# ml4ai/iqlpref

Measured on AMD Instinct MI355X. Metric: iql_grad_steps_per_sec, higher is better.
Workload: dtype bf16; 1 GPU; IQL antmaze-medium-diverse-v2 shapes (S=29 A=8 H=256), 1M-transition device replay, batch 256, one seed per GPU; batch=256, buffer_rows=1000000, graph_unroll=0, graph_launches_per_block=0, eager_steps_per_block=1390

## Files before the change

iqlpref_amd/csrc/api.hip:

```cpp
#include <hip/hip_runtime.h>

#include <algorithm>
#include <cmath>
#include <cstdarg>
#include <cstdio>
#include <cstdlib>
#include <cstring>
#include <new>
#include <vector>

#include "../../include/iqlhip.h"
#include "common.h"
#include "iql_deep.h"
#include "iql_step.h"
#include "step_math.h"

namespace iqlhip {
struct DeepTrainer;
bool deep_shape_ok(const iqlhip_trainer_config &, int n_hidden, const char **why);
hipError_t deep_create(DeepTrainer **, const iqlhip_trainer_config &, int n_hidden, const iqlhip_arenas &,
                       const int64_t *offsets);
void deep_destroy(DeepTrainer *);
hipError_t deep_sync_weights(DeepTrainer *, hipStream_t);
const DeepDesc &deep_desc(const DeepTrainer *);
// ... 726 lines not shown
    TrainNet &N = D.net[n];
    N.in_dim = indim[n], N.k1pad = k1pad[n], N.out_dim = outdim[n], N.out_pad = outpad[n];
    N.has_target = n < E;
    for (int k = 0; k < 3; ++k) {
      N.off_w[k] = L.off[n * 6 + 2 * k];
      N.off_b[k] = L.off[n * 6 + 2 * k + 1];
      N.toff_w[k] = N.has_target ? N.off_w[k] : -1;
      N.toff_b[k] = N.has_target ? N.off_b[k] : -1;
    }
    N.wc[0] = carve<char>(p, (size_t)H * k1pad[n] * es);
    N.wc[1] = carve<char>(p, (size_t)H * H * es);
    N.wc[2] = carve<char>(p, (size_t)outpad[n] * H * es);
    if (N.has_target) {
      N.tc[0] = carve<char>(p, (size_t)H * k1pad[n] * es);
      N.tc[1] = carve<char>(p, (size_t)H * H * es);
      N.tc[2] = carve<char>(p, (size_t)outpad[n] * H * es);
    }
    N.w2ct = carve<char>(p, (size_t)H * H * es);
    N.w3t = carve<char>(p, (size_t)H * outpad[n] * es);
  }
  D.xT = carve<char>(p, (size_t)2 * D.xrows * D.BP * es);
  D.rd = carve<float>(p, (size_t)B * 2);
  D.actf = carve<float>(p, (size_t)B * A);
  D.hT = carve<char>(p, (size_t)NT * 2 * H * D.BP * es);
  D.dz1T = carve<char>(p, (size_t)NT * H * D.BP * es);
  D.dz2T = carve<char>(p, (size_t)NT * H * D.BP * es);
  D.dz3T = carve<char>(p, (size_t)NT * D.opmax * D.BP * es);
  D.outs = carve<float>(p, (size_t)layer2_parts(H) * B * D.OUTW);
  D.lossp = carve<float>(p, (size_t)NT * (B / 16));
  D.lsp = carve<float>(p, (size_t)(B / 16) * A);
  D.ls_snap = carve<float>(p, (size_t)A);
  t->batch_rows = carve<float>(p, (size_t)B * stride);
  D.stage_rows = carve<float>(p, (size_t)B * stride);
  D.stage_stride = stride;
  D.next_off = iqlhip_replay_next_offset(S, A);
  D.prefetch = !getenv("IQLHIP_NO_PREFETCH") ? 1 : 0;
  t->own_dargs = t->dargs = carve<DevArgs>(p, 1);
  t->own_dctr = t->dctr = carve<DevCtr>(p, 1);
  t->own_ddesc = t->ddesc = carve<TrainerDesc>(p, 1);
  t->own_ditems = t->ditems = carve<UpdItem>(p, n_slots);

  for (int n_ = 0; n_ < NT; ++n_)
  for (auto &it : t->net_items[n_]) {
    const TrainNet &N = D.net[it.net];
    const int L = it.layer;
    it.Odim = (L == 2) ? N.out_dim : H;
    it.Idim = (L == 0) ? N.in_dim : H;
    it.Opad = (L == 2) ? N.out_pad : H;
    it.Kw = (L == 0) ? N.k1pad : H;
    it.has_target = N.has_target;
    it.group = it.net == D.net_v ? 1 : (it.net == D.net_a ? 2 : 0);
    it.off_w = N.off_w[L], it.off_b = N.off_b[L], it.toff_w = N.toff_w[L], it.toff_b = N.toff_b[L];

    it.wc = N.wc[L], it.tc = N.has_target ? N.tc[L] : nullptr, it.w2ct = (L == 1) ? N.w2ct : nullptr;
    it.w3t = (L == 2) ? N.w3t : nullptr;
    const size_t plane = (size_t)H * D.BP * es;
    it.Xsrc = (L == 0) ? D.xT : reinterpret_cast<char *>(D.hT) + (size_t)(it.net * 2 + (L - 1)) * plane;
    it.Zsrc = (L == 0)   ? reinterpret_cast<char *>(D.dz1T) + (size_t)it.net * plane
              : (L == 1) ? reinterpret_cast<char *>(D.dz2T) + (size_t)it.net * plane
                         : reinterpret_cast<char *>(D.dz3T) + (size_t)it.net * D.opmax * D.BP * es;
  }
  std::vector<UpdItem> items;
  {
    std::vector<UpdItem> per_xcd[8];
    deal_items(t, 0, 1, per_xcd);
    items = flatten_table(per_xcd, 0, nullptr, (size_t)(B + 15) / 16);
  }
  if (items.size() != n_slots || hipMemcpy(t->ditems, items.data(), items.size() * sizeof(UpdItem), hipMemcpyHostToDevice) !=
      hipSuccess) {
    (void)hipFree(t->ws);
    delete t;
    return fail(IQLHIP_ERR_HIP, "hipMemcpy of the work items failed");
  }

  auto mk = [&](int f, int net, bool target, int in_off, int out_col, int slot) {
    FwdNet &F = D.fwd[f];
    const TrainNet &N = D.net[net];
    F.w1c = target ? N.tc[0] : N.wc[0];
    F.w2c = target ? N.tc[1] : N.wc[1];
    F.w3c = target ? N.tc[2] : N.wc[2];
    const float *base = target ? ar->target : ar->params;
    F.b1 = base + N.off_b[0], F.b2 = base + N.off_b[1], F.b3 = base + N.off_b[2];
    F.in_off = in_off, F.in_dim = N.in_dim, F.k1pad = N.k1pad;
    F.out_dim = N.out_dim, F.out_pad = N.out_pad, F.out_col = out_col;
    F.train_slot = slot;
    F.tanh_out = net == D.net_a;
    F.dropout = (net == D.net_a) && D.has_dropout;
    F.stage = f == 0;
  };
  for (int e = 0; e < E; ++e) mk(e, e, false, 0, e, e);
  mk(E, D.net_v, false, 0, D.out_v, D.net_v);
  mk(E + 1, D.net_a, false, 0, D.out_mean, D.net_a);
  for (int e = 0; e < E; ++e) mk(E + 2 + e, e, true, 0, D.out_qt + e, -1);
  mk(2 * E + 2, D.net_v, false, D.next_off, D.out_nv, -1);

  if (hipMemcpy(t->ddesc, &t->D, sizeof(TrainerDesc), hipMemcpyHostToDevice) != hipSuccess) {
    (void)hipFree(t->ws);
    delete t;
    return fail(IQLHIP_ERR_HIP, "hipMemcpy of the descriptor failed");
  }
  *out = t;
  return 0;
}

extern "C" int iqlhip_trainer_destroy(iqlhip_trainer *t) {
  if (!t) return 0;
  if (t->group) return fail(IQLHIP_ERR_INVALID, "trainer is a member of a group: destroy the group first");
  t->queue.destroy();
// ... 943 lines not shown
```

iqlpref_amd/csrc/iql_step.h:

```cpp
#pragma once
#include <stdint.h>

namespace iqlhip {

constexpr int MAX_CRITICS = 8;
constexpr int MAX_TRAIN = MAX_CRITICS + 2;
constexpr int MAX_FWD = 2 * MAX_CRITICS + 3;

struct FwdNet {
  const void *w1c, *w2c, *w3c;
  const float *b1, *b2, *b3;
  int32_t in_off;
  int32_t in_dim, k1pad;
  int32_t out_dim, out_pad;
  int32_t out_col;
  int32_t train_slot;
  int32_t tanh_out;
  int32_t dropout;
  int32_t stage;
};

struct TrainNet {
  int64_t off_w[3], off_b[3];
  int64_t toff_w[3], toff_b[3];
// ... 27 lines not shown
  float *actf;
  void *hT;
  void *dz1T;
  void *dz2T;
  void *dz3T;
  float *outs;
  float *lossp;
  float *lsp;
  float *ls_snap;
  float *params, *exp_avg, *exp_avg_sq, *target, *grads;
  int64_t off_log_std;
  unsigned long long *dbg;
  double beta1, beta2, eps;
  int64_t t_max;
  FwdNet fwd[MAX_FWD];
  TrainNet net[MAX_TRAIN];
};

struct DevArgs {
  const float *rows;
  int64_t n_rows;
  int32_t row_stride;
  int32_t idx_mode;
  const int64_t *idx;
  const uint8_t *drop_keep;
  float *losses_out;
  int64_t base_step;
  double lr_q, lr_v, lr_a_base;
  int64_t n_steps;
  uint64_t generation;
  const int32_t *n_valid;
};

struct AdamCoef {
  float one_m_b1, b2, one_m_b2, neg_step[3], bc2_sqrt, eps;
  float inv_bc2_sqrt, pad_;
};

struct DevCtr {
  int64_t ctr[2];
  int64_t coef_step;
  AdamCoef coef;
  float last_losses[4];
  double loss_sum[4];
};

struct UpdItem {
  int32_t net, layer;
  int32_t o0, i0;
  int32_t Odim, Idim;
  int32_t Opad, Kw;
  int32_t has_target, group;
  int64_t off_w, off_b, toff_w, toff_b;
  void *wc, *tc, *w2ct;
  void *w3t;
  const void *Xsrc, *Zsrc;
};

}
```

iqlpref_amd/csrc/iql_step.hip:

```cpp
#include "common.h"
#include "iql_step.h"
#include "step_math.h"

namespace iqlhip {

constexpr int SLAB = 16;

#ifdef IQL_STAMPS
#define STAMP(kern, slot)                                                                   \
  do {                                                                                      \
    if (D.dbg && threadIdx.x == 0 && blockIdx.x < 512) {                                                      \
      unsigned long long *d_ = D.dbg + (((size_t)(kern) * 512 + blockIdx.x) * 8 + (slot)) * 2; \
      d_[0] = wall_clock64();                                                               \
      d_[1] = clock64();                                                                    \
    }                                                                                       \
  } while (0)
#else
#define STAMP(kern, slot) \
  do {                    \
  } while (0)
#endif

template <class T>
__device__ __forceinline__ void pin_s(T v) {
// ... 274 lines not shown
          }
        }
      }
    }
  }
  STAMP(0, 5);
}

template <bool BF16>
__device__ __forceinline__ void stage_rows16(const TrainerDesc &D, const DevArgs &A, int64_t step, int row0,
                                             int row_step, int tid) {
  using P = Prec<BF16>;
  using T = typename P::T;
  const int rr = tid >> 4, l16 = tid & 15;
  const int B = D.B, nq = D.stage_stride >> 2, S = D.S, SA = D.S + D.A, nkb = D.BP / P::KM;
  T *const xT = reinterpret_cast<T *>(D.xT) + (size_t)(step & 1) * D.xrows * D.BP;
  for (int row = row0 + rr; row < B; row += row_step) {
    int64_t ix;
    if (A.idx_mode == 1)
      ix = ldg(A.idx + (size_t)(step - A.base_step) * B + row);
    else if (A.idx_mode == 2)
      ix = row;
    else
      ix = philox_index(D.seed, (uint64_t)step, (uint32_t)row, (uint64_t)A.n_rows);
    ix = ix < 0 ? 0 : (ix >= A.n_rows ? A.n_rows - 1 : ix);
    const float *src = A.rows + (size_t)ix * A.row_stride;
    float *dst = D.stage_rows + (size_t)row * D.stage_stride;
    for (int c = l16; c < nq; c += 16) {
      const float4 v4 = __builtin_bit_cast(float4, ldg16(src + 4 * c));
      stg16(dst + 4 * c, v4);
      const float v[4] = {v4.x, v4.y, v4.z, v4.w};
#pragma unroll
      for (int e = 0; e < 4; ++e) {
        const int col = 4 * c + e;
        if (col < SA) stg(xT + fidx<P>(col, row, nkb), P::from_f32(v[e]));
        if (col >= S && col < SA) stg(D.actf + (size_t)row * D.A + (col - S), v[e]);
        if (col >= SA && col < SA + 2) stg(D.rd + (size_t)row * 2 + (col - SA), v[e]);
      }
    }
  }
}

template <bool BF16>
__global__ __launch_bounds__(256) void k_stage(const TrainerDesc *__restrict__ Dp,
                                               const DevArgs *__restrict__ Ap,
                                               const DevCtr *__restrict__ Cp) {
  Dp += blockIdx.y, Ap += blockIdx.y, Cp += blockIdx.y;
  stage_rows16<BF16>(*Dp, *Ap, Cp->ctr[0], blockIdx.x * 16, gridDim.x * 16, threadIdx.x);
}

__device__ __forceinline__ void write_adam_coef(const TrainerDesc &D, const DevArgs &A, int64_t t1,
                                                AdamCoef *out);

template <bool BF16, int H>
struct FCfg {
  using P = Prec<BF16>;
  static constexpr int TPW = H / 64;
  static constexpr int SPL = TPW >= 4 ? 4 : TPW;
  static constexpr int HQ = H / SPL;
  static constexpr int NK2 = H / P::KM;
  static constexpr int NK3 = HQ / P::KM;
  static constexpr int NK1 = BF16 ? 4 : 8;
  static constexpr int HP = H + P::EPV;
  static constexpr int HQP = HQ + P::EPV;
  static_assert(HQ == 64, "one 16-column tile per wave and part");
};

template <bool BF16, int H, int MT, int PW>
__global__ __launch_bounds__(256, 3) void k_forward(const TrainerDesc *__restrict__ Dp,
                                                 const DevArgs *__restrict__ Ap,
                                                 const DevCtr *__restrict__ Cp, const int nsl_,
                                                 const int nfwd_) {
  using C = FCfg<BF16, H>;
  using P = Prec<BF16>;
  using T = typename P::T;
  constexpr int ROWS = 16 * MT, TPW = C::TPW, SPL = C::SPL, HP = C::HP, HQP = C::HQP;
  constexpr int NPG = SPL / PW;
  static_assert(SPL % PW == 0 && PW <= 2, "parts per work-group: 1 or 2, dividing the parts");
  Dp += blockIdx.y, Ap += blockIdx.y, Cp += blockIdx.y;
  const TrainerDesc &D = *Dp;
  const int idx_ = blockIdx.x >> 3;
  const int per_job = nsl_ * NPG;
  const int fnet = (idx_ / per_job) * 8 + (blockIdx.x & 7);
  const int rest = idx_ % per_job;
  const int slab = rest / NPG;
  const int part0 = __builtin_amdgcn_readfirstlane((rest % NPG) * PW);
  if (fnet > nfwd_) return;
  if (fnet == nfwd_) {
    if (rest == 0 && threadIdx.x == 0) {
      STAMP(0, 0);
      write_adam_coef(D, *Ap, Cp->ctr[0] + 1, const_cast<AdamCoef *>(&Cp->coef));
      const_cast<DevCtr *>(Cp)->coef_step = Cp->ctr[0] + 1;
      STAMP(0, 5);
    }
    if (rest == 0 && !D.deterministic && (int)threadIdx.x < D.A)
      stg(D.ls_snap + threadIdx.x, ldg(D.params + D.off_log_std + threadIdx.x));
    return;
  }
  const FwdNet N = D.fwd[fnet];
  const int B = D.B, BP = D.BP, OUTW = D.OUTW, k1max = D.k1max;
  const float *const stage = D.stage_rows;
  const unsigned sstride = (unsigned)D.stage_stride;
  float *const g_outs = D.outs;
  void *const g_hT = D.hT;
  const int64_t step = Cp->ctr[0];
  extern __shared__ __attribute__((aligned(16))) char smem[];
  const int tid = threadIdx.x, lane = tid & 63;
  const int wave = __builtin_amdgcn_readfirstlane(tid >> 6);
  const int r = lane & 15, q = lane >> 4;
  const int K1P = k1max + P::EPV;
  T *xs = reinterpret_cast<T *>(smem);
  T *h1 = xs + ROWS * K1P;
  T *h2 = h1 + ROWS * HP;
  STAMP(0, 0);

  const int rr = tid >> 4, l16 = tid & 15;
  const int lim4 = round_up(N.in_dim, 4) - 4;
  float4 xq[MT][2];
#pragma unroll
  for (int m = 0; m < MT; ++m) {
    const int row_ = slab * ROWS + 16 * m + rr;
    const unsigned row = (unsigned)(row_ < B ? row_ : B - 1);
    const float *src = stage + N.in_off;
#pragma unroll
    for (int j = 0; j < 2; ++j) {
      const int c = 4 * l16 + 64 * j;
      xq[m][j] = __builtin_bit_cast(float4, ldg16(src + (row * sstride + (unsigned)(c < lim4 ? c : lim4))));
    }
  }
  const int nk1 = N.k1pad / P::KM;
  const int nt3 = N.out_pad / 16;
  const int tile2 = part0 * 4 + wave;
  float bias1[TPW], bias3[2];
  {
    const float *b1w = N.b1 + 16 * (wave * TPW);
#pragma unroll
    for (int jj = 0; jj < TPW; ++jj) bias1[jj] = ldg(b1w + 16 * jj + r);
  }
  float bias2[PW];
#pragma unroll
  for (int j = 0; j < PW; ++j) bias2[j] = ldg(N.b2 + 16 * (tile2 + 4 * j) + r);
#pragma unroll
  for (int jt = 0; jt < 2; ++jt)
    bias3[jt] = ldg(N.b3 + (16 * jt + r < N.out_dim ? 16 * jt + r : N.out_dim - 1));
  uint4 w1[C::NK1][TPW], w2[PW][C::NK2], w3[PW][C::NK3][2];
  auto load_w2 = [&]() {
#pragma unroll
    for (int j = 0; j < PW; ++j) {
      const T *W2w = reinterpret_cast<const T *>(N.w2c) + (size_t)(tile2 + 4 * j) * C::NK2 * 64 * P::EPV;
#pragma unroll
      for (int ks = 0; ks < C::NK2; ++ks) w2[j][ks] = ldg16(W2w + ks * 64 * P::EPV + lane * P::EPV);
    }
  };
  auto load_w3 = [&]() {
#pragma unroll
    for (int j = 0; j < PW; ++j) {
      const T *W3w = reinterpret_cast<const T *>(N.w3c) + (size_t)((part0 + j) * C::NK3) * 64 * P::EPV;
#pragma unroll
      for (int ks = 0; ks < C::NK3; ++ks)
// ... 188 lines not shown

  for (int pr = wave; pr < MT * PW; pr += 4) {
    const int m = pr % MT, j = pr / MT;
    const T *h2j = h2 + j * ROWS * HQP;
    f32x4 acc3[2] = {f32x4{0.f, 0.f, 0.f, 0.f}, f32x4{0.f, 0.f, 0.f, 0.f}};
#pragma unroll
    for (int ks = 0; ks < C::NK3; ++ks) {
      const uint4 a = *reinterpret_cast<const uint4 *>(h2j + (16 * m + r) * HQP + ks * P::KM + P::EPV * q);
#pragma unroll
      for (int jt = 0; jt < 2; ++jt) {
        if (jt < nt3) {
          if constexpr (PW == 1) {
            P::mma(a, w3[0][ks][jt], acc3[jt]);
          } else {
            if (j == 0) P::mma(a, w3[0][ks][jt], acc3[jt]);
            else P::mma(a, w3[PW - 1][ks][jt], acc3[jt]);
          }
        }
      }
    }
    float *outp = g_outs + (size_t)(part0 + j) * B * OUTW;
    const int row0 = slab * ROWS + 16 * m + 4 * q;
#pragma unroll
    for (int jt = 0; jt < 2; ++jt) {
      const int col = 16 * jt + r;
      if (jt < nt3 && col < N.out_dim && row0 < B) {
        const float bias = part0 + j == 0 ? P::round(bias3[jt]) : 0.f;
        outs_store4<false>(outp, (size_t)(N.out_col + col) * B + row0,
                           make_float4(acc3[jt][0] + bias, acc3[jt][1] + bias, acc3[jt][2] + bias, acc3[jt][3] + bias));
      }
    }
  }
  STAMP(0, 5);
}

template <int H, bool DROP>
__global__ __launch_bounds__(512, 1) void k_forward_tp(const TrainerDesc *__restrict__ Dp,
                                                        const DevArgs *__restrict__ Ap,
                                                        const DevCtr *__restrict__ Cp, const int nsl_,
                                                        const int nfwd_) {
  using C = FCfg<true, H>;
  using P = Prec<true>;
  using T = typename P::T;
  constexpr int ROWS = 64, MT = ROWS / 16, NW = 8;
  constexpr int TPW = H / (16 * NW);
  constexpr int SPL = C::SPL, HP = C::HP, NK2 = C::NK2, NK3 = C::NK3;
  static_assert(H == 256 && TPW == 2 && SPL == 4, "k_forward_tp is built for H = 256");
  Dp += blockIdx.y, Ap += blockIdx.y, Cp += blockIdx.y;
  const TrainerDesc &D = *Dp;
  const int idx_ = blockIdx.x >> 3;
  const int fnet = (idx_ / nsl_) * 8 + (blockIdx.x & 7);
  const int slab = idx_ % nsl_;
  if (fnet > nfwd_) return;
  if (fnet == nfwd_) {
    if (slab == 0 && threadIdx.x == 0) {
      STAMP(0, 0);
      write_adam_coef(D, *Ap, Cp->ctr[0] + 1, const_cast<AdamCoef *>(&Cp->coef));
      const_cast<DevCtr *>(Cp)->coef_step = Cp->ctr[0] + 1;
      STAMP(0, 5);
    }
    if (slab == 0 && !D.deterministic && (int)threadIdx.x < D.A)
      stg(D.ls_snap + threadIdx.x, ldg(D.params + D.off_log_std + threadIdx.x));
    return;
  }
  const FwdNet N = D.fwd[fnet];
  const int B = D.B, BP = D.BP, OUTW = D.OUTW, k1max = D.k1max;
  const float *const stage = D.stage_rows;
  const unsigned sstride = (unsigned)D.stage_stride;
  float *const g_outs = D.outs;
  void *const g_hT = D.hT;
  const int64_t step = Cp->ctr[0];
  extern __shared__ __attribute__((aligned(16))) char smem[];
  const int tid = threadIdx.x, lane = tid & 63;
  const int wave = __builtin_amdgcn_readfirstlane(tid >> 6);
  const int r = lane & 15, q = lane >> 4;
  const int K1P = k1max + P::EPV;
  T *xs = reinterpret_cast<T *>(smem);
  T *h1 = xs + ROWS * K1P;
  T *h2 = h1 + ROWS * HP;
  STAMP(0, 0);

  const int rr = tid >> 3, l8 = tid & 7;
  const int lim4 = round_up(N.in_dim, 4) - 4;
  float4 xq[4];
  {
    const int row_ = slab * ROWS + rr;
    const unsigned row = (unsigned)(row_ < B ? row_ : B - 1);
    const float *src = stage + N.in_off;
#pragma unroll
    for (int j = 0; j < 4; ++j) {
      const int c = 4 * l8 + 32 * j;
      xq[j] = __builtin_bit_cast(float4, ldg16(src + (row * sstride + (unsigned)(c < lim4 ? c : lim4))));
    }
  }
  const int nk1 = N.k1pad / P::KM;
  const int nt3 = N.out_pad / 16;
  const int tile0 = wave * TPW;
  const int part = tile0 / 4;
  float bias1[TPW], bias2[TPW], bias3[2];
#pragma unroll
  for (int jj = 0; jj < TPW; ++jj) {
    bias1[jj] = ldg(N.b1 + 16 * (tile0 + jj) + r);
    bias2[jj] = ldg(N.b2 + 16 * (tile0 + jj) + r);
  }
#pragma unroll
  for (int jt = 0; jt < 2; ++jt)
    bias3[jt] = ldg(N.b3 + (16 * jt + r < N.out_dim ? 16 * jt + r : N.out_dim - 1));
  uint4 w1[C::NK1][TPW], w2[TPW][NK2], w3[NK3][2];
  {
    const T *W1w = reinterpret_cast<const T *>(N.w1c) + (size_t)tile0 * nk1 * 64 * P::EPV;
#pragma unroll
    for (int ks = 0; ks < C::NK1; ++ks) {
      if (ks < nk1) {
#pragma unroll
        for (int jj = 0; jj < TPW; ++jj)
          w1[ks][jj] = ldg16(W1w + (size_t)(jj * nk1 + ks) * 64 * P::EPV + lane * P::EPV);
      }
    }
  }
  auto load_w23 = [&]() {
#pragma unroll
    for (int jj = 0; jj < TPW; ++jj) {
      const T *W2w = reinterpret_cast<const T *>(N.w2c) + (size_t)(tile0 + jj) * NK2 * 64 * P::EPV;
#pragma unroll
      for (int ks = 0; ks < NK2; ++ks) w2[jj][ks] = ldg16(W2w + ks * 64 * P::EPV + lane * P::EPV);
// ... 850 lines not shown
      for (int s = 0; s < nslab; ++s) g += sred[nl + s * D.A + tid];
      const int64_t o = D.off_log_std + tid;
      const float lsc = fminf(fmaxf(ls, -20.f), 2.f);
      g = g * expf(lsc) * ((ls >= -20.f && ls <= 2.f) ? 1.f : 0.f);
      float p = ls;
      adam_apply<BF16>(p, pm, pv, g, coef, coef.neg_step[2]);
      stg(D.params + o, p), stg(D.exp_avg + o, pm), stg(D.exp_avg_sq + o, pv);
      if (D.grads) stg(D.grads + o, g);
    }
    if (tid >= 64 && tid < 64 + nt) {
      const int n = tid - 64;
      float s = 0.f;
      for (int k = 0; k < nslab; ++k) s += sred[n * nslab + k];
      int nv = B;
      if constexpr (!BF16) nv = VALID_ROWS(A.n_valid, A, t1 - 1, B);
      sred[nl + na + n] = s / (float)nv;
    }
    __syncthreads();
    if (tid == 64) {
      const float vl = sred[nl + na + D.net_v];
      float ql = 0.f;
      for (int e = 0; e < D.E; ++e) ql += sred[nl + na + e];
      ql = ql / (float)D.E;
      const float al = sred[nl + na + D.net_a];
      Cp->last_losses[0] = vl, Cp->last_losses[1] = ql, Cp->last_losses[2] = al;
      Cp->loss_sum[0] += vl, Cp->loss_sum[1] += ql, Cp->loss_sum[2] += al;
      if (A.losses_out) {
        float *lo = A.losses_out + (size_t)(t1 - 1 - A.base_step) * 3;
        stg(lo, vl), stg(lo + 1, ql), stg(lo + 2, al);
      }
      Cp->ctr[0] = t1;
    }
    STAMP(2, 4);
    return;
  }

  if (it.net < 0) {
    if (D.prefetch && (A.idx_mode == 0 || (A.idx_mode == 1 && t1 - A.base_step < A.n_steps)))
      stage_rows16<BF16>(D, A, t1, it.o0 * (UT / 16), it.i0 * (UT / 16), tid);
    return;
  }
  const int L = it.layer;
  const int Odim = it.Odim, Idim = it.Idim, Kw = it.Kw, Opad = it.Opad;
  const int Ipad = round_up(Idim, 16);
  const int o0 = it.o0, i0 = it.i0;
  const float neg_step =
      it.group == 0 ? coef.neg_step[0] : (it.group == 1 ? coef.neg_step[1] : coef.neg_step[2]);
  const bool has_target = it.has_target != 0;
  const int nk = BP / P::KM;
  const int kh = (BF16 && nk >= 16) ? (nk / (2 * UKC)) * UKC : nk;
  const bool ksplit = kh < nk;
  pin_s(D.tau), pin_s(D.one_m_tau), pin_s(D.polyak_convex);
  pin_s(it.off_w), pin_s(it.toff_w), pin_s(it.off_b), pin_s(it.toff_b), pin_s(it.wc), pin_s(it.tc);
  pin_s(it.w2ct), pin_s(it.Xsrc), pin_s(it.Zsrc), pin_s(Kw), pin_s(neg_step);
  pin_s(coef.one_m_b1), pin_s(coef.b2), pin_s(coef.one_m_b2), pin_s(coef.bc2_sqrt), pin_s(coef.eps);
  pin_s(coef.inv_bc2_sqrt);

  if (L == 0) {
    const int TLD = Ipad + 4;
    const int64_t fbase = it.off_w + (int64_t)o0 * Idim, tbase = it.toff_w + (int64_t)o0 * Idim;
    constexpr int UNE = LAT ? (USR * UMAXI + UT - 1) / UT : 1;
    constexpr int UN4 = LAT ? 1 : (USR * UMAXI / 4 + UT - 1) / UT;
    const int n_el = USR * Idim, n4 = n_el >> 2;
    float pf[UNE], mf[UNE], vf[UNE], tf[UNE];
    float4 pf4[UN4], mf4[UN4], vf4[UN4], tf4[UN4];
    float pb, mb, vb, tb;
    auto load_state = [&]() {
      if constexpr (LAT) {
#pragma unroll
        for (int k = 0; k < UNE; ++k) {
          const int e = tid + UT * k;
          const int ec = e < n_el ? e : n_el - 1;
          pf[k] = ldg(g_params + fbase + ec);
          mf[k] = ldg(g_m + fbase + ec);
          vf[k] = ldg(g_v + fbase + ec);
          tf[k] = ldg((has_target ? g_target + tbase : g_params + fbase) + ec);
        }
      } else {
#pragma unroll
        for (int k = 0; k < UN4; ++k) {
          if (UT * k < n4) {
            const int e4 = tid + UT * k;
            const int ec = 4 * (e4 < n4 ? e4 : n4 - 1);
            pf4[k] = __builtin_bit_cast(float4, ldg16(g_params + fbase + ec));
            mf4[k] = __builtin_bit_cast(float4, ldg16(g_m + fbase + ec));
            vf4[k] = __builtin_bit_cast(float4, ldg16(g_v + fbase + ec));
            tf4[k] = __builtin_bit_cast(float4, ldg16((has_target ? g_target + tbase : g_params + fbase) + ec));
          }
        }
      }
      const int ob_ = o0 + (tid & (USR - 1));
      const int64_t eb = it.off_b + ob_;
      pb = ldg(g_params + eb), mb = ldg(g_m + eb), vb = ldg(g_v + eb);
      tb = ldg((has_target ? g_target + it.toff_b : g_params + it.off_b) + ob_);
    };
    if constexpr (LAT) load_state();
    STAMP(2, 1);
    const T *Xsrc = reinterpret_cast<const T *>(it.Xsrc) + (size_t)((t1 - 1) & 1) * D.xrows * BP;
    const T *Zsrc = reinterpret_cast<const T *>(it.Zsrc);
    const int nit = Ipad >> 4;
    const int wo = wave % UOT, th = wave / UOT;
    constexpr int NT = UNIT / UWPO;
    f32x4 acc[NT];
#pragma unroll
    for (int t = 0; t < NT; ++t) acc[t] = f32x4{0.f, 0.f, 0.f, 0.f};
    float bsum = 0.f;
    constexpr int TB = NT < 2 ? NT : 2;
// ... 308 lines not shown
          }
          __builtin_amdgcn_sched_barrier(0);
          if (ks + GIF < UKC) issue(k0, ks + GIF);
        }
      };
      chunk(kbeg, true);
#pragma unroll 1
      for (int k0 = kbeg + UKC; k0 < kend; k0 += UKC) chunk(k0, false);
      __builtin_amdgcn_sched_barrier(0);
      load_state();
      float *const tdst = half ? tile2 : tile;
#pragma unroll
      for (int b = 0; b < GNB; ++b)
#pragma unroll
        for (int c = 0; c < GNI; ++c)
          *reinterpret_cast<f32x4 *>(&tdst[(16 * GNB * gw + 16 * b + r) * ULD + 16 * c + 4 * q]) = acc[b][c];
      if (wave_bias) {
#pragma unroll
        for (int b = 0; b < GNB; ++b) {
          float bs = bsum[b];
          bs = xor32_sum(xor16_sum(bs));
          if (q == 0) (half ? bgrad2 : bgrad)[16 * GNB * gw + 16 * b + r] = bs;
        }
      }
    }
  }
  __syncthreads();
  STAMP(2, 3);

  T *wc = reinterpret_cast<T *>(it.wc);
  T *tc = reinterpret_cast<T *>(it.tc);
  const int nkw = Kw / P::KM;
#pragma unroll
  for (int ps = 0; ps < UNP; ++ps) {
    const int ol = tr + URPP * ps, o = o0 + ol, i = i0 + tc4;
    const float4 g4 = *reinterpret_cast<const float4 *>(&tile[ol * ULD + tc4]);
    float g[4] = {g4.x, g4.y, g4.z, g4.w};
    if constexpr (!LAT) {
      if (ksplit) {
        const float4 h4 = *reinterpret_cast<const float4 *>(&tile2[ol * ULD + tc4]);
        g[0] += h4.x, g[1] += h4.y, g[2] += h4.z, g[3] += h4.w;
      }
    }
    float p[4] = {pw[ps][0], pw[ps][1], pw[ps][2], pw[ps][3]};
    float m[4] = {mw[ps][0], mw[ps][1], mw[ps][2], mw[ps][3]};
    float v[4] = {vw[ps][0], vw[ps][1], vw[ps][2], vw[ps][3]};
    float tv[4] = {tw[ps][0], tw[ps][1], tw[ps][2], tw[ps][3]};
#pragma unroll
    for (int k = 0; k < 4; ++k) {
      g[k] = P::round(g[k]);
      adam_apply<BF16>(p[k], m[k], v[k], g[k], coef, neg_step);
      if (has_target) tv[k] = polyak(D, tv[k], p[k]);
    }
    if (L == 1) *reinterpret_cast<float4 *>(&tile[ol * ULD + tc4]) = make_float4(p[0], p[1], p[2], p[3]);
    const bool copies_from_lds = !LAT && L == 1;
    if (copies_from_lds && has_target)
      *reinterpret_cast<float4 *>(&tile2[ol * ULD + tc4]) = make_float4(tv[0], tv[1], tv[2], tv[3]);
    if (o < Odim && i < Idim) {
      const int64_t e = it.off_w + (int64_t)o * Idim + i;
      const int64_t te = it.toff_w + (int64_t)o * Idim + i;
      state_store(g_params, e, make_float4(p[0], p[1], p[2], p[3]));
      state_store(g_m, e, make_float4(m[0], m[1], m[2], m[3]));
      state_store(g_v, e, make_float4(v[0], v[1], v[2], v[3]));
      if (g_grads) stg16(g_grads + e, make_float4(g[0], g[1], g[2], g[3]));
      if (has_target) state_store(g_target, te, make_float4(tv[0], tv[1], tv[2], tv[3]));
      if (!copies_from_lds) {
        store4T<BF16>(wc + fidx<P>(o, i, nkw), p);
        if (has_target) store4T<BF16>(tc + fidx<P>(o, i, nkw), tv);
      }
      if (L == 2) {
        T *w3t = reinterpret_cast<T *>(it.w3t);
#pragma unroll
        for (int k = 0; k < 4; ++k) stg(w3t + (size_t)(i + k) * Opad + o, P::from_f32(p[k]));
      }
    }
  }
  STAMP(2, 5);
  if (do_bias && tid < UTO && o0 + tid < Odim) {
    const int64_t e = it.off_b + o0 + tid;
    float gb = bgrad[tid];
    if constexpr (!LAT) {
      if (ksplit) gb += bgrad2[tid];
    }
    const float g = P::round(gb);
    adam_apply<BF16>(pb, mb, vb, g, coef, neg_step);
    stg(g_params + e, pb), stg(g_m + e, mb), stg(g_v + e, vb);
    if (g_grads) stg(g_grads + e, g);
    if (has_target) stg(g_target + it.toff_b + o0 + tid, polyak(D, tb, pb));
  }
  STAMP(2, 6);
  if (L == 1) {
    __syncthreads();
    if constexpr (!LAT) {
      static_assert(LAT || (UT == 256 && UTO == 64 && UTI == 32), "one pass of 8-element stores covers the tile");
      {
        const int ol = tid >> 2, c8 = (tid & 3) * 8;
        const float4 a0 = *reinterpret_cast<const float4 *>(&tile[ol * ULD + c8]);
        const float4 a1 = *reinterpret_cast<const float4 *>(&tile[ol * ULD + c8 + 4]);
        const float pv8[8] = {a0.x, a0.y, a0.z, a0.w, a1.x, a1.y, a1.z, a1.w};
        copy_store8<BF16>(wc, fidx<P>(o0 + ol, i0 + c8, nkw), fidx<P>(o0 + ol, i0 + c8 + 4, nkw), pv8);
        if (has_target) {
          const float4 t0 = *reinterpret_cast<const float4 *>(&tile2[ol * ULD + c8]);
          const float4 t1 = *reinterpret_cast<const float4 *>(&tile2[ol * ULD + c8 + 4]);
          const float tv8[8] = {t0.x, t0.y, t0.z, t0.w, t1.x, t1.y, t1.z, t1.w};
          copy_store8<BF16>(tc, fidx<P>(o0 + ol, i0 + c8, nkw), fidx<P>(o0 + ol, i0 + c8 + 4, nkw), tv8);
        }
      }
      {
        const int il = tid & (UTI - 1), o8 = (tid >> 5) * 8;
        float pv8[8];
#pragma unroll
        for (int k = 0; k < 8; ++k) pv8[k] = tile[(o8 + k) * ULD + il];
        copy_store8<BF16>(reinterpret_cast<T *>(it.w2ct), fidx<P>(i0 + il, o0 + o8, H / P::KM),
                          fidx<P>(i0 + il, o0 + o8 + 4, H / P::KM), pv8);
      }
      STAMP(2, 4);
      return;
    }
#pragma unroll
    for (int ps = 0; ps < (UTO / 4) / (UT / UTI); ++ps) {
      const int il = tid & (UTI - 1), o4 = ((tid >> 5) + (UT / UTI) * ps) * 4;
      float pv4[4];
#pragma unroll
      for (int k = 0; k < 4; ++k) pv4[k] = tile[(o4 + k) * ULD + il];
      store4T<BF16>(reinterpret_cast<T *>(it.w2ct) + fidx<P>(i0 + il, o0 + o4, H / P::KM), pv4);
    }
  }
  STAMP(2, 4);
}

template <bool BF16, int H, bool PRE, int PW, bool NV = false>
__global__ __launch_bounds__(256, PRE ? 1 : (PW > 1 ? (BF16 ? 4 : 2) : (BF16 ? 6 : 3)))
void k_backward(const TrainerDesc *__restrict__ Dp, const DevArgs *__restrict__ Ap, DevCtr *__restrict__ Cp,
                const int nslab, const int ntrain) {
  extern __shared__ __attribute__((aligned(16))) char smem[];
  backward_body<BF16, H, PRE, PW, NV>(Dp + blockIdx.y, Ap + blockIdx.y, Cp + blockIdx.y, (int)blockIdx.x, smem, nslab,
                                      ntrain);
}

template <bool BF16, bool LAT>
__global__ __launch_bounds__(LAT ? 512 : 256, LAT ? 2 : (BF16 ? 4 : 3)) void k_update(const TrainerDesc *__restrict__ Dp,
                                                             const DevArgs *__restrict__ Ap,
                                                             DevCtr *__restrict__ Cp,
                                                             const UpdItem *__restrict__ items, int n_items) {
  if ((int)blockIdx.x > n_items) return;
  update_body<BF16, LAT, (LAT ? 512 : 256)>(Dp + blockIdx.y, Ap + blockIdx.y, Cp + blockIdx.y,
                         items + (size_t)blockIdx.y * n_items, n_items, (int)blockIdx.x);
}

template <bool BF16>
__global__ void k_sync_weights(const TrainerDesc *__restrict__ Dp) {
  const TrainerDesc &D = *Dp;
  using P = Prec<BF16>;
  using T = typename P::T;
  const int net = blockIdx.y;
  if (net >= D.ntrain) return;
  const TrainNet &N = D.net[net];
  const int H = D.H;
  for (int L = 0; L < 3; ++L) {
    const int Odim = (L == 2) ? N.out_dim : H;
    const int Idim = (L == 0) ? N.in_dim : H;
    const int Kw = (L == 0) ? N.k1pad : H;
    const int total = Odim * Idim;
    for (int e = blockIdx.x * blockDim.x + threadIdx.x; e < total; e += gridDim.x * blockDim.x) {
      const int o = e / Idim, i = e - o * Idim;
      const float p = ldg(D.params + N.off_w[L] + e);
      stg(reinterpret_cast<T *>(N.wc[L]) + fidx<P>(o, i, Kw / P::KM), P::from_f32(p));
      if (L == 1) stg(reinterpret_cast<T *>(N.w2ct) + fidx<P>(i, o, H / P::KM), P::from_f32(p));
      if (L == 2) stg(reinterpret_cast<T *>(N.w3t) + (size_t)i * N.out_pad + o, P::from_f32(p));
      if (N.has_target)
        stg(reinterpret_cast<T *>(N.tc[L]) + fidx<P>(o, i, Kw / P::KM),
            P::from_f32(ldg(D.target + N.toff_w[L] + e)));
    }
  }
}

size_t infer_smem_bytes(bool bf16, int H, int k1max) {
  const int es = bf16 ? 2 : 4, epv = bf16 ? 8 : 4;
  return (size_t)SLAB * (k1max + epv) * es + 2 * (size_t)SLAB * (H + epv) * es + 4 * 2 * 64 * 4 * 4;
}
size_t fwd_smem_bytes(bool bf16, int H, int k1max, int mt, int pw) {
  const int es = bf16 ? 2 : 4, epv = bf16 ? 8 : 4;
  return (size_t)16 * mt * ((k1max + epv) + (H + epv) + pw * (64 + epv)) * es;
}
size_t bwd_smem_bytes(bool bf16, int H) {
  const int es = bf16 ? 2 : 4, epv = bf16 ? 8 : 4;
  return (size_t)SLAB * (H + epv) * es + 3 * SLAB * 32 * 4 + SLAB * 4 + SLAB * FIN_LD * 4;
}
int fwd_row_tiles(int B, int n_seeds) {
  const int64_t rows = (int64_t)B * n_seeds;
  if (rows >= 512 && B % 32 == 0) return 2;
  return 1;
}
int layer2_parts(int H) { return H >= 256 ? 4 : H / 64; }
int fwd_parts_per_wg(int B, int H, int n_seeds) {
  return ((int64_t)B * n_seeds >= 1024 && layer2_parts(H) % 2 == 0) ? 2 : 1;
}

#define DISPATCH_H(BF, HH, CALL)                 \
  do {                                           \
    if (BF) {                                    \
      if (HH == 256) { CALL(true, 256); }        \
      else if (HH == 128) { CALL(true, 128); }   \
      else { CALL(true, 64); }                   \
    } else {                                     \
      if (HH == 256) { CALL(false, 256); }       \
      else if (HH == 128) { CALL(false, 128); }  \
      else { CALL(false, 64); }                  \
    }                                            \
  } while (0)

bool use_tp(bool bf16, const TrainerDesc &D, int n_seeds, bool backward) {
  if (!bf16 || D.H != 256 || D.B % 64 != 0) return false;
  const int64_t fwd_wgs = (int64_t)D.nfwd * (D.B / 64) * n_seeds, bwd_wgs = (int64_t)D.ntrain * (D.B / 32) * n_seeds;
  const bool fwd_tp = fwd_wgs >= 72 && fwd_wgs <= 256;
  return backward ? (fwd_tp && bwd_wgs >= 144 && bwd_wgs <= 256) : fwd_tp;
}
hipError_t prepare_step_kernels() {
  hipError_t e = hipFuncSetAttribute(reinterpret_cast<const void *>(k_forward_tp<256, false>),
                                     hipFuncAttributeMaxDynamicSharedMemorySize, 160 * 1024);
  if (e != hipSuccess) return e;
  return hipFuncSetAttribute(reinterpret_cast<const void *>(k_forward_tp<256, true>),
                             hipFuncAttributeMaxDynamicSharedMemorySize, 160 * 1024);
}
size_t fwd_tp_smem_bytes(int H, int k1max) { return (size_t)64 * ((k1max + 8) + 2 * (H + 8)) * 2; }
size_t bwd_smem_bytes(bool bf16, int H);

hipError_t launch_forward(bool bf16, const TrainerDesc &D, const TrainerDesc *dD, const DevArgs *a,
                          const DevCtr *c, int n_seeds, hipStream_t st) {
  if (use_tp(bf16, D, n_seeds, false)) {
    const int nsl64 = D.B / 64;
    const int grid = 8 * ((D.nfwd + 1 + 7) / 8) * nsl64;
    if (D.has_dropout)
      hipLaunchKernelGGL((k_forward_tp<256, true>), dim3(grid, n_seeds), dim3(512), fwd_tp_smem_bytes(256, D.k1max), st,
                         dD, a, c, nsl64, D.nfwd);
    else
      hipLaunchKernelGGL((k_forward_tp<256, false>), dim3(grid, n_seeds), dim3(512), fwd_tp_smem_bytes(256, D.k1max), st,
                         dD, a, c, nsl64, D.nfwd);
    return hipGetLastError();
  }
  const int mt = fwd_row_tiles(D.B, n_seeds), nsl = (D.B + 16 * mt - 1) / (16 * mt);
  const int pw = fwd_parts_per_wg(D.B, D.H, n_seeds);
  const int grid = 8 * ((D.nfwd + 1 + 7) / 8) * nsl * (layer2_parts(D.H) / pw);
  const size_t sm = fwd_smem_bytes(bf16, D.H, D.k1max, mt, pw);
#define LAUNCH_F(BF, HH, MTV, PWV)                                                                            \
  hipLaunchKernelGGL((k_forward<BF, HH, MTV, PWV>), dim3(grid, n_seeds), dim3(256), sm, st, dD, a, c, nsl, D.nfwd)
#define CALL(BF, HH)                                                   \
  do {                                                                 \
    if constexpr (HH >= 128) {                                         \
      if (pw == 2) {                                                   \
        if (mt == 2) LAUNCH_F(BF, HH, 2, 2);                           \
        else LAUNCH_F(BF, HH, 1, 2);                                   \
        break;                                                         \
      }                                                                \
    }                                                                  \
    if (mt == 2) LAUNCH_F(BF, HH, 2, 1);                               \
    else LAUNCH_F(BF, HH, 1, 1);                                       \
  } while (0)
  DISPATCH_H(bf16, D.H, CALL);
#undef CALL
#undef LAUNCH_F
  return hipGetLastError();
}
int bwd_parts_per_wg(int B, int H, int n_seeds) {
  return ((int64_t)B * n_seeds >= 512 && layer2_parts(H) % 2 == 0) ? 2 : 1;
}
hipError_t launch_backward(bool bf16, const TrainerDesc &D, const TrainerDesc *dD, const DevArgs *a,
                           DevCtr *c, int n_seeds, hipStream_t st, bool counts) {
  if (use_tp(bf16, D, n_seeds, true)) {
    const int nslab32 = D.B / 32;
    const int nxn = (D.ntrain <= 4 && nslab32 % 2 == 0) ? 2 : 1;
    const int grid = 8 * ((D.ntrain * nxn + 7) / 8) * (nslab32 / nxn);
    hipLaunchKernelGGL((k_backward_tp<256>), dim3(grid, n_seeds), dim3(512), 2 * bwd_smem_bytes(true, 256), st, dD, a, c,
                       nslab32, D.ntrain, nxn);
    return hipGetLastError();
  }
  const int pw = bwd_parts_per_wg(D.B, D.H, n_seeds);
  const int grid = 8 * ((layer2_parts(D.H) / pw * D.ntrain + 7) / 8) * (D.B / SLAB);
// ... 88 lines not shown
```

Measured before the change: 67100 steps/s.

## Move transposed weight copies from update kernel into spare forward work-groups

The update kernel no longer writes the transposed layer-2 weights (w2ct) or the layer-3 transpose (w3t). The spare forward job (fnet == nfwd) now rebuilds them from the compact weight copies at the start of the next step, spreading the blocks over otherwise idle work-groups and transposing through LDS. This shortens the update kernel's tail and removes its scattered strided stores. In exchange the forward kernel does extra global reads and writes, and the forward kernels that consume w2ct/w3t must not read them before the copy finishes, which looks like an ordering risk.

Result: no change. 67070 steps/s (-0.0%).

```diff
diff --git a/iqlpref_amd/csrc/api.hip b/iqlpref_amd/csrc/api.hip
--- a/iqlpref_amd/csrc/api.hip
+++ b/iqlpref_amd/csrc/api.hip
@@ -802,8 +802,7 @@
     it.group = it.net == D.net_v ? 1 : (it.net == D.net_a ? 2 : 0);
     it.off_w = N.off_w[L], it.off_b = N.off_b[L], it.toff_w = N.toff_w[L], it.toff_b = N.toff_b[L];
 
-    it.wc = N.wc[L], it.tc = N.has_target ? N.tc[L] : nullptr, it.w2ct = (L == 1) ? N.w2ct : nullptr;
-    it.w3t = (L == 2) ? N.w3t : nullptr;
+    it.wc = N.wc[L], it.tc = N.has_target ? N.tc[L] : nullptr;
     const size_t plane = (size_t)H * D.BP * es;
     it.Xsrc = (L == 0) ? D.xT : reinterpret_cast<char *>(D.hT) + (size_t)(it.net * 2 + (L - 1)) * plane;
     it.Zsrc = (L == 0)   ? reinterpret_cast<char *>(D.dz1T) + (size_t)it.net * plane
diff --git a/iqlpref_amd/csrc/iql_step.h b/iqlpref_amd/csrc/iql_step.h
--- a/iqlpref_amd/csrc/iql_step.h
+++ b/iqlpref_amd/csrc/iql_step.h
@@ -103,8 +103,7 @@
   int32_t Opad, Kw;
   int32_t has_target, group;
   int64_t off_w, off_b, toff_w, toff_b;
-  void *wc, *tc, *w2ct;
-  void *w3t;
+  void *wc, *tc;
   const void *Xsrc, *Zsrc;
 };
 
diff --git a/iqlpref_amd/csrc/iql_step.hip b/iqlpref_amd/csrc/iql_step.hip
--- a/iqlpref_amd/csrc/iql_step.hip
+++ b/iqlpref_amd/csrc/iql_step.hip
@@ -350,6 +350,151 @@
 __device__ __forceinline__ void write_adam_coef(const TrainerDesc &D, const DevArgs &A, int64_t t1,
                                                 AdamCoef *out);
 
+template <bool BF16>
+constexpr int fwd_copy_tile_bytes() {
+  return 64 * (64 + Prec<BF16>::EPV) * (int)sizeof(typename Prec<BF16>::T);
+}
+constexpr int FWD_TP_COPY_U = 7;
+
+template <bool BF16, int H, int NT, int U>
+__device__ __forceinline__ void fwd_copies(const TrainerDesc &D, const int ntrain, const int wg, const int nwg,
+                                           char *smem) {
+  using P = Prec<BF16>;
+  using T = typename P::T;
+  constexpr int EPV = P::EPV, KM = P::KM, LD = 64 + EPV;
+  constexpr int KS = 64 / KM;
+  constexpr int NF = 4 * KS;
+  constexpr int NWV = NT / 64;
+  constexpr int FR = NF / NWV;
+  static_assert(NF % NWV == 0 && FR >= 1, "a block's fragments are dealt evenly over the waves");
+  constexpr int nb = H / 64, nb2 = nb * nb, nk = H / KM;
+  const int tid = threadIdx.x, lane = tid & 63;
+  const int wave = __builtin_amdgcn_readfirstlane(tid >> 6);
+  const int nblocks = ntrain * nb2, nitems = nblocks + ntrain;
+  const int n_mine = wg < nblocks ? (nblocks - wg + nwg - 1) / nwg : 0;
+  const int npass = (n_mine + U - 1) / U;
+  T *const tiles = reinterpret_cast<T *>(smem);
+
+  auto load_pass = [&](const int pass, uint4(&w)[U][FR]) {
+#pragma unroll
+    for (int u = 0; u < U; ++u) {
+      const int id_ = wg + nwg * (pass * U + u);
+      const int id = id_ < nblocks ? id_ : nblocks - 1;
+      const int net = id / nb2, b = id % nb2, ob = b / nb, ib = b % nb;
+      const T *src = reinterpret_cast<const T *>(D.net[net].wc[1]);
+#pragma unroll
+      for (int f = 0; f < FR; ++f) {
+        const int g = wave + NWV * f, ft = g / KS, fk = g % KS;
+        w[u][f] = ldg16(src + frag_off<P>(4 * ob + ft, ib * KS + fk, nk, lane));
+      }
+    }
+  };
+  uint4 cur[U][FR];
+  if (npass > 0) load_pass(0, cur);
+
+#pragma unroll 1
+  for (int pass = 0; pass < npass; ++pass) {
+    uint4 nxt[U][FR];
+#pragma unroll
+    for (int u = 0; u < U; ++u)
+#pragma unroll
+      for (int f = 0; f < FR; ++f) nxt[u][f] = cur[u][f];
+    if (pass + 1 < npass) load_pass(pass + 1, nxt);
+#pragma unroll
+    for (int u = 0; u < U; ++u)
+#pragma unroll
+      for (int f = 0; f < FR; ++f) {
+        const int g = wave + NWV * f, ft = g / KS, fk = g % KS;
+        *reinterpret_cast<uint4 *>(tiles + (size_t)u * 64 * LD + (16 * ft + (lane & 15)) * LD + KM * fk + EPV * (lane >> 4)) =
+            cur[u][f];
+      }
+    __syncthreads();
+#pragma unroll
+    for (int u = 0; u < U; ++u) {
+      const int id = wg + nwg * (pass * U + u);
+      if (id < nblocks) {
+        const int net = id / nb2, b = id % nb2, ob = b / nb, ib = b % nb;
+        const void *dst = D.net[net].w2ct;
+        const T *tu = tiles + (size_t)u * 64 * LD;
+#pragma unroll
+        for (int f = 0; f < FR; ++f) {
+          const int g = wave + NWV * f, ft = g / KS, fk = g % KS;
+          const T *col = tu + (KM * fk + EPV * (lane >> 4)) * LD + 16 * ft + (lane & 15);
+          uint4 o;
+          if constexpr (BF16) {
+            o.x = (uint32_t)col[0] | ((uint32_t)col[LD] << 16), o.y = (uint32_t)col[2 * LD] | ((uint32_t)col[3 * LD] << 16);
+            o.z = (uint32_t)col[4 * LD] | ((uint32_t)col[5 * LD] << 16);
+            o.w = (uint32_t)col[6 * LD] | ((uint32_t)col[7 * LD] << 16);
+          } else {
+            o = __builtin_bit_cast(uint4, make_float4(col[0], col[LD], col[2 * LD], col[3 * LD]));
+          }
+          stg16_wt(dst, (uint32_t)(frag_off<P>(4 * ib + ft, ob * KS + fk, nk, lane) * sizeof(T)),
+                   __builtin_bit_cast(float4, o));
+        }
+      }
+    }
+    __syncthreads();
+#pragma unroll
+    for (int u = 0; u < U; ++u)
+#pragma unroll
+      for (int f = 0; f < FR; ++f) cur[u][f] = nxt[u][f];
+  }
+
+  constexpr int LDW = H + EPV;
+  constexpr int NFW = H / KM;
+  constexpr int FW = (NFW + NWV - 1) / NWV;
+  constexpr int PPI = 16 / EPV;
+  constexpr int NPC = (H * PPI + NT - 1) / NT;
+  static_assert(16 * LDW * (int)sizeof(T) <= fwd_copy_tile_bytes<BF16>(), "a w3t tile fits a block's LDS region");
+  const int first3 = nblocks <= wg ? wg : wg + (nblocks - wg + nwg - 1) / nwg * nwg;
+#pragma unroll 1
+  for (int id = first3; id < nitems; id += nwg) {
+    const TrainNet &N = D.net[id - nblocks];
+    const T *src = reinterpret_cast<const T *>(N.wc[2]);
+    const void *dst = N.w3t;
+    const int out_pad = N.out_pad;
+#pragma unroll 1
+    for (int jt = 0; 16 * jt < out_pad; ++jt) {
+      uint4 w[FW];
+#pragma unroll
+      for (int f = 0; f < FW; ++f) {
+        const int g = wave + NWV * f;
+        w[f] = ldg16(src + frag_off<P>(jt, g < NFW ? g : NFW - 1, nk, lane));
+      }
+#pragma unroll
+      for (int f = 0; f < FW; ++f) {
+        const int g = wave + NWV * f;
+        if (g < NFW) *reinterpret_cast<uint4 *>(tiles + (lane & 15) * LDW + KM * g + EPV * (lane >> 4)) = w[f];
+      }
+      __syncthreads();
+#pragma unroll
+      for (int j = 0; j < NPC; ++j) {
+        const int pc = tid + NT * j;
+        if (pc < H * PPI) {
+          const int i = pc / PPI, po = pc % PPI;
+          const T *col = tiles + (EPV * po) * LDW + i;
+          uint4 o;
+          if constexpr (BF16) {
+            o.x = (uint32_t)col[0] | ((uint32_t)col[LDW] << 16), o.y = (uint32_t)col[2 * LDW] | ((uint32_t)col[3 * LDW] << 16);
+            o.z = (uint32_t)col[4 * LDW] | ((uint32_t)col[5 * LDW] << 16);
+            o.w = (uint32_t)col[6 * LDW] | ((uint32_t)col[7 * LDW] << 16);
+          } else {
+            o = __builtin_bit_cast(uint4, make_float4(col[0], col[LDW], col[2 * LDW], col[3 * LDW]));
+          }
+          stg16_wt(dst, (uint32_t)((i * out_pad + 16 * jt + EPV * po) * sizeof(T)), __builtin_bit_cast(float4, o));
+        }
+      }
+      __syncthreads();
+    }
+  }
+}
+
+template <bool BF16, int H, int NT, int U>
+__device__ __attribute__((noinline)) void fwd_copies_call(const TrainerDesc &D, const int ntrain, const int wg,
+                                                          const int nwg, char *smem) {
+  fwd_copies<BF16, H, NT, U>(D, ntrain, wg, nwg, smem);
+}
+
 template <bool BF16, int H>
 struct FCfg {
   using P = Prec<BF16>;
@@ -384,9 +529,19 @@
   const int slab = rest / NPG;
   const int part0 = __builtin_amdgcn_readfirstlane((rest % NPG) * PW);
   if (fnet > nfwd_) return;
+  extern __shared__ __attribute__((aligned(16))) char smem[];
   if (fnet == nfwd_) {
+    STAMP(0, 0);
+    if (rest > 0 || per_job == 1) {
+      const int ntrain = (nfwd_ + 1) >> 1;
+      const int cw = per_job == 1 ? 0 : rest - 1, ncw = per_job == 1 ? 1 : per_job - 1;
+      if constexpr (BF16 && H == 256 && MT * PW == 4)
+        fwd_copies_call<BF16, H, 256, 1>(D, ntrain, cw, ncw, smem);
+      else
+        fwd_copies<BF16, H, 256, 1>(D, ntrain, cw, ncw, smem);
+      STAMP(0, 6);
+    }
     if (rest == 0 && threadIdx.x == 0) {
-      STAMP(0, 0);
       write_adam_coef(D, *Ap, Cp->ctr[0] + 1, const_cast<AdamCoef *>(&Cp->coef));
       const_cast<DevCtr *>(Cp)->coef_step = Cp->ctr[0] + 1;
       STAMP(0, 5);
@@ -402,7 +557,6 @@
   float *const g_outs = D.outs;
   void *const g_hT = D.hT;
   const int64_t step = Cp->ctr[0];
-  extern __shared__ __attribute__((aligned(16))) char smem[];
   const int tid = threadIdx.x, lane = tid & 63;
   const int wave = __builtin_amdgcn_readfirstlane(tid >> 6);
   const int r = lane & 15, q = lane >> 4;
@@ -697,9 +851,14 @@
   const int fnet = (idx_ / nsl_) * 8 + (blockIdx.x & 7);
   const int slab = idx_ % nsl_;
   if (fnet > nfwd_) return;
+  extern __shared__ __attribute__((aligned(16))) char smem[];
   if (fnet == nfwd_) {
+    STAMP(0, 0);
+    if (slab > 0 || nsl_ == 1) {
+      fwd_copies<true, H, 512, FWD_TP_COPY_U>(D, (nfwd_ + 1) >> 1, nsl_ == 1 ? 0 : slab - 1, nsl_ == 1 ? 1 : nsl_ - 1, smem);
+      STAMP(0, 6);
+    }
     if (slab == 0 && threadIdx.x == 0) {
-      STAMP(0, 0);
       write_adam_coef(D, *Ap, Cp->ctr[0] + 1, const_cast<AdamCoef *>(&Cp->coef));
       const_cast<DevCtr *>(Cp)->coef_step = Cp->ctr[0] + 1;
       STAMP(0, 5);
@@ -715,7 +874,6 @@
   float *const g_outs = D.outs;
   void *const g_hT = D.hT;
   const int64_t step = Cp->ctr[0];
-  extern __shared__ __attribute__((aligned(16))) char smem[];
   const int tid = threadIdx.x, lane = tid & 63;
   const int wave = __builtin_amdgcn_readfirstlane(tid >> 6);
   const int r = lane & 15, q = lane >> 4;
@@ -1672,7 +1830,7 @@
   const bool ksplit = kh < nk;
   pin_s(D.tau), pin_s(D.one_m_tau), pin_s(D.polyak_convex);
   pin_s(it.off_w), pin_s(it.toff_w), pin_s(it.off_b), pin_s(it.toff_b), pin_s(it.wc), pin_s(it.tc);
-  pin_s(it.w2ct), pin_s(it.Xsrc), pin_s(it.Zsrc), pin_s(Kw), pin_s(neg_step);
+  pin_s(it.Xsrc), pin_s(it.Zsrc), pin_s(Kw), pin_s(neg_step);
   pin_s(coef.one_m_b1), pin_s(coef.b2), pin_s(coef.one_m_b2), pin_s(coef.bc2_sqrt), pin_s(coef.eps);
   pin_s(coef.inv_bc2_sqrt);
 
@@ -2087,10 +2245,11 @@
       adam_apply<BF16>(p[k], m[k], v[k], g[k], coef, neg_step);
       if (has_target) tv[k] = polyak(D, tv[k], p[k]);
     }
-    if (L == 1) *reinterpret_cast<float4 *>(&tile[ol * ULD + tc4]) = make_float4(p[0], p[1], p[2], p[3]);
     const bool copies_from_lds = !LAT && L == 1;
-    if (copies_from_lds && has_target)
-      *reinterpret_cast<float4 *>(&tile2[ol * ULD + tc4]) = make_float4(tv[0], tv[1], tv[2], tv[3]);
+    if (copies_from_lds) {
+      *reinterpret_cast<float4 *>(&tile[ol * ULD + tc4]) = make_float4(p[0], p[1], p[2], p[3]);
+      if (has_target) *reinterpret_cast<float4 *>(&tile2[ol * ULD + tc4]) = make_float4(tv[0], tv[1], tv[2], tv[3]);
+    }
     if (o < Odim && i < Idim) {
       const int64_t e = it.off_w + (int64_t)o * Idim + i;
       const int64_t te = it.toff_w + (int64_t)o * Idim + i;
@@ -2103,11 +2262,6 @@
         store4T<BF16>(wc + fidx<P>(o, i, nkw), p);
         if (has_target) store4T<BF16>(tc + fidx<P>(o, i, nkw), tv);
       }
-      if (L == 2) {
-        T *w3t = reinterpret_cast<T *>(it.w3t);
-#pragma unroll
-        for (int k = 0; k < 4; ++k) stg(w3t + (size_t)(i + k) * Opad + o, P::from_f32(p[k]));
-      }
     }
   }
   STAMP(2, 5);
@@ -2124,44 +2278,24 @@
     if (has_target) stg(g_target + it.toff_b + o0 + tid, polyak(D, tb, pb));
   }
   STAMP(2, 6);
-  if (L == 1) {
-    __syncthreads();
-    if constexpr (!LAT) {
+  if constexpr (!LAT) {
+    if (L == 1) {
+      __syncthreads();
       static_assert(LAT || (UT == 256 && UTO == 64 && UTI == 32), "one pass of 8-element stores covers the tile");
-      {
-        const int ol = tid >> 2, c8 = (tid & 3) * 8;
-        const float4 a0 = *reinterpret_cast<const float4 *>(&tile[ol * ULD + c8]);
-        const float4 a1 = *reinterpret_cast<const float4 *>(&tile[ol * ULD + c8 + 4]);
-        const float pv8[8] = {a0.x, a0.y, a0.z, a0.w, a1.x, a1.y, a1.z, a1.w};
-        copy_store8<BF16>(wc, fidx<P>(o0 + ol, i0 + c8, nkw), fidx<P>(o0 + ol, i0 + c8 + 4, nkw), pv8);
-        if (has_target) {
-          const float4 t0 = *reinterpret_cast<const float4 *>(&tile2[ol * ULD + c8]);
-          const float4 t1 = *reinterpret_cast<const float4 *>(&tile2[ol * ULD + c8 + 4]);
-          const float tv8[8] = {t0.x, t0.y, t0.z, t0.w, t1.x, t1.y, t1.z, t1.w};
-          copy_store8<BF16>(tc, fidx<P>(o0 + ol, i0 + c8, nkw), fidx<P>(o0 + ol, i0 + c8 + 4, nkw), tv8);
-        }
-      }
-      {
-        const int il = tid & (UTI - 1), o8 = (tid >> 5) * 8;
-        float pv8[8];
-#pragma unroll
-        for (int k = 0; k < 8; ++k) pv8[k] = tile[(o8 + k) * ULD + il];
-        copy_store8<BF16>(reinterpret_cast<T *>(it.w2ct), fidx<P>(i0 + il, o0 + o8, H / P::KM),
-                          fidx<P>(i0 + il, o0 + o8 + 4, H / P::KM), pv8);
+      const int ol = tid >> 2, c8 = (tid & 3) * 8;
+      const float4 a0 = *reinterpret_cast<const float4 *>(&tile[ol * ULD + c8]);
+      const float4 a1 = *reinterpret_cast<const float4 *>(&tile[ol * ULD + c8 + 4]);
+      const float pv8[8] = {a0.x, a0.y, a0.z, a0.w, a1.x, a1.y, a1.z, a1.w};
+      copy_store8<BF16>(wc, fidx<P>(o0 + ol, i0 + c8, nkw), fidx<P>(o0 + ol, i0 + c8 + 4, nkw), pv8);
+      if (has_target) {
+        const float4 t0 = *reinterpret_cast<const float4 *>(&tile2[ol * ULD + c8]);
+        const float4 t1 = *reinterpret_cast<const float4 *>(&tile2[ol * ULD + c8 + 4]);
+        const float tv8[8] = {t0.x, t0.y, t0.z, t0.w, t1.x, t1.y, t1.z, t1.w};
+        copy_store8<BF16>(tc, fidx<P>(o0 + ol, i0 + c8, nkw), fidx<P>(o0 + ol, i0 + c8 + 4, nkw), tv8);
       }
       STAMP(2, 4);
-      return;
-    }
-#pragma unroll
-    for (int ps = 0; ps < (UTO / 4) / (UT / UTI); ++ps) {
-      const int il = tid & (UTI - 1), o4 = ((tid >> 5) + (UT / UTI) * ps) * 4;
-      float pv4[4];
-#pragma unroll
-      for (int k = 0; k < 4; ++k) pv4[k] = tile[(o4 + k) * ULD + il];
-      store4T<BF16>(reinterpret_cast<T *>(it.w2ct) + fidx<P>(i0 + il, o0 + o4, H / P::KM), pv4);
-    }
-  }
-  STAMP(2, 4);
+    }
+  }
 }
 
 template <bool BF16, int H, bool PRE, int PW, bool NV = false>
@@ -2216,7 +2350,9 @@
 }
 size_t fwd_smem_bytes(bool bf16, int H, int k1max, int mt, int pw) {
   const int es = bf16 ? 2 : 4, epv = bf16 ? 8 : 4;
-  return (size_t)16 * mt * ((k1max + epv) + (H + epv) + pw * (64 + epv)) * es;
+  const size_t eval = (size_t)16 * mt * ((k1max + epv) + (H + epv) + pw * (64 + epv)) * es;
+  const size_t copy = (size_t)(bf16 ? fwd_copy_tile_bytes<true>() : fwd_copy_tile_bytes<false>());
+  return eval > copy ? eval : copy;
 }
 size_t bwd_smem_bytes(bool bf16, int H) {
   const int es = bf16 ? 2 : 4, epv = bf16 ? 8 : 4;
@@ -2259,6 +2395,8 @@
                              hipFuncAttributeMaxDynamicSharedMemorySize, 160 * 1024);
 }
 size_t fwd_tp_smem_bytes(int H, int k1max) { return (size_t)64 * ((k1max + 8) + 2 * (H + 8)) * 2; }
+static_assert(FWD_TP_COPY_U * fwd_copy_tile_bytes<true>() <= 64 * (8 + 2 * (256 + 8)) * 2,
+              "the spare job's blocks fit the LDS of a k_forward_tp work-group");
 size_t bwd_smem_bytes(bool bf16, int H);
 
 hipError_t launch_forward(bool bf16, const TrainerDesc &D, const TrainerDesc *dD, const DevArgs *a,
```
